# astra-vision/PaSCo

Measured on AMD Instinct MI355X. Metric: scenes/sec (256x256x32, ~10% occ) PaSCo MIMO-3, higher is better.
Workload: dtype f32 (conv products as 3 x f16 split MFMA, fp32 accumulate)

## Files before the change

### pasco_amd/csrc/conv_dma.hip

```cpp
#include <mutex>
#include <stdlib.h>

#include <hip/hip_runtime.h>
#include "ph_common.h"
#ifdef PH_DEV
__device__ unsigned long long g_dma_trace[64 * 8];
#define DMA_STAMP(i)                                                                                              \
  do {                                                                                                            \
    if ((a.ablate & 0x80) && threadIdx.x == 0 && blockIdx.x < 64 && blockIdx.y == 0)                              \
      g_dma_trace[blockIdx.x * 8 + (i)] = __builtin_readcyclecounter();                                           \
  } while (0)
#else
#define DMA_STAMP(i) do { } while (0)
#endif
#define H2_STAMP(i) DMA_STAMP(i)
#include "conv_h2_common.h"

#ifdef PH_DEV
extern "C" int ph_dma_trace_read(unsigned long long *host_out) {
  return hipMemcpyFromSymbol(host_out, HIP_SYMBOL(g_dma_trace), sizeof(g_dma_trace)) == hipSuccess ? 0 : 2;
}
#endif
constexpr int DMA_DENSE_KVOL = 100;
constexpr int DMA_KMAX = 32;
// ... 38 lines not shown
  const int cout = a.cout;
  const int nchunks = a.cpad >> 5;
  const int kper = (a.kvol + a.ksplit - 1) / a.ksplit;
  int k_begin = (int)blockIdx.y * kper;
  const int k_end = (k_begin + kper < a.kvol) ? k_begin + kper : a.kvol;
  int kcount = k_end > k_begin ? k_end - k_begin : 0;
  int kstride = 1;
  if (a.kvol > DMA_DENSE_KVOL && a.tile_k == nullptr && a.ksplit > 1 && !PH_ABLATE(a, 4)) {
    kstride = a.ksplit;
    k_begin = (int)blockIdx.y;
    kcount = k_begin < a.kvol ? (a.kvol - k_begin + kstride - 1) / kstride : 0;
  }
  if (a.tile_k != nullptr) {
    k_begin = a.tile_k[row_tile];
    if (k_begin < 0) return;
    kcount = 1;
  }
  int nstages = kcount * nchunks;
  const uint32_t rsb = 4u * (uint32_t)a.cpad;

  f32x16 acc[TM][TN];
#pragma unroll
  for (int i = 0; i < TM; ++i)
#pragma unroll
    for (int j = 0; j < TN; ++j)
#pragma unroll
      for (int r = 0; r < 16; ++r) acc[i][j][r] = 0.f;

  if (nstages > 0) {
    int *idx_lds = reinterpret_cast<int *>(lds + 2 * STAGE);
    for (int i = tid; i < kcount * BM; i += NT) {
      const int k = i / BM, r = i - k * BM;
      const int64_t row = m0 + r;
      int idx = -1;
      if (row < a.n_out) idx = a.tile_k ? a.nbr[row] : (a.nbr ? a.nbr[(int64_t)(k_begin + k * kstride) * a.nbr_stride + row] : (int)row);
      idx_lds[k * BM + (r % RPP) * 4 + (r / RPP)] = idx;
    }
    asm volatile("s_waitcnt vmcnt(0) lgkmcnt(0)" ::: "memory");
    __builtin_amdgcn_s_barrier();
    DMA_STAMP(7);

    static_assert(BM >= 2 * DMA_KMAX + 4, "the stage list fits one offset slot of the index table");
    int *kmap = idx_lds + (DMA_KMAX - 1) * BM;
    const bool compact = a.kvol > DMA_DENSE_KVOL && a.tile_k == nullptr && !PH_ABLATE(a, 4);
    if (compact) {
      int *kflag = kmap + DMA_KMAX;
      for (int k = wave; k < kcount; k += WAVES) {
        bool any = false;
        for (int r = lane; r < BM; r += 64) any |= idx_lds[k * BM + r] >= 0;
        const unsigned long long bal = __ballot(any);
        if (lane == 0) kflag[k] = bal != 0ull ? 1 : 0;
      }
      asm volatile("s_waitcnt lgkmcnt(0)" ::: "memory");
      __builtin_amdgcn_s_barrier();
      if (tid == 0) {
        int nv = 0;
        for (int k = 0; k < kcount; ++k)
          if (kflag[k]) kmap[nv++] = k;
        kflag[DMA_KMAX] = nv;
      }
      asm volatile("s_waitcnt lgkmcnt(0)" ::: "memory");
      __builtin_amdgcn_s_barrier();
      nstages = kflag[DMA_KMAX] * nchunks;
    }
    if (nstages > 0) {

    const int l_j = tid & 7;
    const int l_r = tid >> 3;
    const uint32_t sj16 = (uint32_t)((l_j ^ ((l_r >> 1) & 7)) << 4);
    const uint64_t in_base = (uint64_t)reinterpret_cast<uintptr_t>(a.in_split) + sj16;
    const uint64_t zero_src = (uint64_t)reinterpret_cast<uintptr_t>(a.zero) + sj16;
    const uint64_t w_base = (uint64_t)reinterpret_cast<uintptr_t>(a.w_split) + sj16;
    uint32_t boff[B_PASSES];
#pragma unroll
    for (int q = 0; q < B_PASSES; ++q) {
      int n = n0 + l_r + q * RPP;
      n = n < cout ? n : cout - 1;
      boff[q] = (uint32_t)n * rsb;
    }
    const int64_t wslab = (int64_t)cout * rsb;
    static_assert(A_PASSES == 4, "one 16-byte index read per thread and stage");
    typedef int i32x4 __attribute__((ext_vector_type(4)));

    auto stage_kc = [&](int s, int &k, uint32_t &coff) {
      const int sc = s < nstages - 1 ? s : nstages - 1;
      const int kk = sc / nchunks;
      coff = (uint32_t)(sc - kk * nchunks) << 7;
      k = compact ? kmap[kk] : kk;
    };
    auto load_idx = [&](int s) {
      int k;
      uint32_t coff;
      stage_kc(s, k, coff);
      return *reinterpret_cast<const i32x4 *>(idx_lds + k * BM + l_r * 4);
    };
    struct Src {
      uint64_t a[A_PASSES];
      uint64_t w;
    };
    auto prep = [&](int s, const i32x4 &idx, Src &src) {
      int k;
      uint32_t coff;
      stage_kc(s, k, coff);
#pragma unroll
      for (int p = 0; p < A_PASSES; ++p) {
        const int ix = idx[p];
        uint64_t v = in_base + (uint64_t)(uint32_t)(ix < 0 ? 0 : ix) * rsb + coff;
        asm volatile("" : "+v"(v));
        src.a[p] = ix >= 0 ? v : zero_src;
      }
      src.w = w_base + (uint64_t)((int64_t)(k_begin + k * kstride) * wslab) + coff;
    };
    auto fire = [&](const Src &src, int buf) {
      char *abuf = lds + buf * STAGE;
#pragma unroll
      for (int p = 0; p < A_PASSES; ++p) {
        char *dst = abuf + (p * RPP + wave * 8) * 128;
        __builtin_amdgcn_global_load_lds((const __attribute__((address_space(1))) void *)(uintptr_t)src.a[p],
                                         (__attribute__((address_space(3))) void *)dst, 16, 0, 0);
      }
#pragma unroll
      for (int q = 0; q < B_PASSES; ++q) {
        char *dst = abuf + A_BYTES + (q * RPP + wave * 8) * 128;
        __builtin_amdgcn_global_load_lds((const __attribute__((address_space(1))) void *)(uintptr_t)(src.w + boff[q]),
                                         (__attribute__((address_space(3))) void *)dst, 16, 0, 0);
      }
    };

    const int sw = (l31 >> 1) & 7;
    uint32_t xo[2][2];
#pragma unroll
    for (int ks = 0; ks < 2; ++ks)
#pragma unroll
      for (int part = 0; part < 2; ++part) xo[ks][part] = (uint32_t)(((part * 4 + ks * 2 + h) ^ sw) << 4);
    const uint32_t arow = (uint32_t)((wm * TM * 32 + l31) * 128);
    const uint32_t brow = (uint32_t)(A_BYTES + (wn * TN * 32 + l31) * 128);

    struct Frag {
      f16x8 ah[2][TM], al[2][TM], bh[2][TN], bl[2][TN];
    };
    auto readfrag = [&](int buf, Frag &f) {
      const char *base = lds + buf * STAGE;
#pragma unroll
      for (int ks = 0; ks < 2; ++ks) {
#pragma unroll
        for (int i = 0; i < TM; ++i) {
          f.ah[ks][i] = *reinterpret_cast<const f16x8 *>(base + arow + i * 4096 + xo[ks][0]);
          f.al[ks][i] = *reinterpret_cast<const f16x8 *>(base + arow + i * 4096 + xo[ks][1]);
        }
#pragma unroll
        for (int j = 0; j < TN; ++j) {
          f.bh[ks][j] = *reinterpret_cast<const f16x8 *>(base + brow + j * 4096 + xo[ks][0]);
          f.bl[ks][j] = *reinterpret_cast<const f16x8 *>(base + brow + j * 4096 + xo[ks][1]);
        }
      }
    };
    auto mfma = [&](const Frag &f) {
#pragma unroll
      for (int ks = 0; ks < 2; ++ks)
#pragma unroll
        for (int i = 0; i < TM; ++i)
#pragma unroll
          for (int j = 0; j < TN; ++j) {
            acc[i][j] = __builtin_amdgcn_mfma_f32_32x32x16_f16(f.bh[ks][j], f.al[ks][i], acc[i][j], 0, 0, 0);
            acc[i][j] = __builtin_amdgcn_mfma_f32_32x32x16_f16(f.bl[ks][j], f.ah[ks][i], acc[i][j], 0, 0, 0);
            acc[i][j] = __builtin_amdgcn_mfma_f32_32x32x16_f16(f.bh[ks][j], f.ah[ks][i], acc[i][j], 0, 0, 0);
          }
    };
    auto fire_mfma = [&](const Src &src, int buf, const Frag &f) {
      char *abuf = lds + buf * STAGE;
// ... 177 lines not shown
```

### pasco_amd/csrc/conv_f16x3.hip

```cpp
#include <stdio.h>
#include <stdlib.h>

#include "conv_h2_common.h"

template <int BM, int KC, int WM, int WN, int TM, int TN>
__global__ void __launch_bounds__(HV_THREADS) k_conv_f16x3(ConvArgsH a) {
  constexpr int BN = WN * TN * 32;
  constexpr int HKC = KC;
  constexpr int H_LD = KC + 8;
  constexpr int A_TPR = KC / 4;
  constexpr int A_RPP = HV_THREADS / A_TPR;
  constexpr int A_PASSES = BM / A_RPP;
  constexpr int B_SPR = KC / 8;
  constexpr int B_SLOTS = (BN * B_SPR + HV_THREADS - 1) / HV_THREADS;
  static_assert(WM * WN == 4 && WM * TM * 32 == BM, "tile shape");
  static_assert(B_SLOTS >= 1, "loader shape");

  __shared__ __attribute__((aligned(16))) _Float16 Ah[BM * H_LD];
  __shared__ __attribute__((aligned(16))) _Float16 Al[BM * H_LD];
  __shared__ __attribute__((aligned(16))) _Float16 Bh[BN * H_LD];
  __shared__ __attribute__((aligned(16))) _Float16 Bl[BN * H_LD];

  const int nwg = gridDim.x;
  const int cpx = nwg >> 3;
// ... 466 lines not shown
    x = h_act(x * (a.epi_scale ? a.epi_scale[c] : 1.f) + (a.epi_shift ? a.epi_shift[c] : 0.f), a.epi_neg);
    if (a.has_tail) {
      x = x * (a.epi2_scale ? a.epi2_scale[c] : 1.f) + (a.epi2_shift ? a.epi2_shift[c] : 0.f);
      x = h_act(x + r4[q], a.res_neg);
    }
    v[q] = x;
  }
  if (a.out) *reinterpret_cast<float4 *>(a.out + t) = make_float4(v[0], v[1], v[2], v[3]);
  if (a.out_split) {
    float sc[4], sh[4];
#pragma unroll
    for (int q = 0; q < 4; ++q) {
      sc[q] = a.osp_scale ? a.osp_scale[col + q] : 1.f;
      sh[q] = a.osp_shift ? a.osp_shift[col + q] : 0.f;
    }
    const bool obad = emit_split4(v, sc, sh, a.osp_has, a.osp_neg, a.act_pow2,
                                  a.out_split + (row * (a.cout >> 5) + (col >> 5)) * 64 + (col & 31));
    if (a.status != nullptr && obad) atomicOr(a.status, 1);
  }
}

static int ph_launch_splitk_epilogue(const ConvArgsH &args, hipStream_t st) {
  const int64_t total = args.n_out * args.cout;
  hipLaunchKernelGGL(k_splitk_epilogue, dim3((unsigned)((total / 4 + 255) / 256)), dim3(256), 0, st, args);
  PH_LAUNCH_CHECK();
  return 0;
}

static int ph_conv_h_launch(const ConvArgsH &a, const ConvStep &s, hipStream_t st) {
  const bool pre = s.kernel == CONV_K_H2;
  ConvKernelFn k = nullptr;
#define PH_H2(KC_, BM_, WM_, WN_, TM_, TN_)                                                                                    \
  (s.emit ? k_conv_h2<BM_, KC_, WM_, WN_, TM_, TN_, true> : k_conv_h2<BM_, KC_, WM_, WN_, TM_, TN_, false>)
#define PH_H_CASE(BM_, WM_, WN_, TM_, TN_)                                                                                     \
  if (s.bm == BM_) {                                                                                                           \
    if (pre) k = s.kc == 64 ? PH_H2(64, BM_, WM_, WN_, TM_, TN_) : PH_H2(32, BM_, WM_, WN_, TM_, TN_);                         \
    else k = s.kc == 64 ? k_conv_f16x3<BM_, 64, WM_, WN_, TM_, TN_> : k_conv_f16x3<BM_, 32, WM_, WN_, TM_, TN_>;               \
  }
  if (s.bn == 32) {
    PH_H_CASE(128, 4, 1, 1, 1);
  } else if (s.bn == 64) {
    PH_H_CASE(128, 4, 1, 1, 2);
    PH_H_CASE(64, 2, 2, 1, 1);
  } else {
    PH_H_CASE(128, 2, 2, 2, 2);
    PH_H_CASE(64, 2, 2, 1, 2);
    PH_H_CASE(32, 1, 4, 1, 1);
  }
#undef PH_H_CASE
#undef PH_H2
  if (k == nullptr) {
    ph_set_error("conv_fwd(f16x3): no kernel for bm=%d bn=%d", s.bm, s.bn);
    return 1;
  }
  return ph_launch_tiles(k, a, s, st);
}

static ConvKnobs conv_knobs_from_env() {
  ConvKnobs k;
  auto on = [](const char *e, bool dflt) { return e == nullptr ? dflt : atoi(e) != 0; };
  if (const char *e = PH_DEV_ENV("PASCO_CONV_DMA")) {
    k.dma_on = atoi(e) != 0;
    k.dma_all = atoi(e) == 2;
  }
  if (const char *e = PH_DEV_ENV("PASCO_CONV_WIN")) {
    k.win_on = atoi(e) != 0;
    k.win_wide = atoi(e) == 2;
  }
  k.wide_on = on(PH_DEV_ENV("PASCO_CONV_WIDE"), true);
  k.mid_on = on(PH_DEV_ENV("PASCO_CONVH_MID"), true);
  k.rl_on = on(PH_DEV_ENV("PASCO_CONV_RL"), true);
  if (const char *e = PH_DEV_ENV("PASCO_CONVH_CFG")) k.has_cfg = sscanf(e, "%d,%d", &k.cfg_bm, &k.cfg_kc) >= 1;
  if (const char *e = PH_DEV_ENV("PASCO_CONVH_KSPLIT")) {
    k.has_ksplit = true;
    k.ksplit = atoi(e);
  }
  k.ksplit_model = on(PH_DEV_ENV("PASCO_CONVH_KSPLIT_MODEL"), true);
  k.tail_on = on(PH_DEV_ENV("PASCO_CONV_TAIL"), true);
  k.dma_inter = on(PH_DEV_ENV("PASCO_CONV_DMA_INTER"), true);
  k.wop2 = on(PH_DEV_ENV("PASCO_WOP"), true);
  if (const char *e = PH_DEV_ENV("PASCO_CONV_LIN")) k.lin_on = atoi(e);
  if (const char *e = PH_DEV_ENV("PASCO_GRID_KS")) k.grid_ks = atoi(e);
  k.grid_upw = on(PH_DEV_ENV("PASCO_GRID_UPW"), true);
  return k;
}
#ifdef PH_DEV
static ConvKnobs &conv_knobs() {
  static ConvKnobs k = conv_knobs_from_env();
  return k;
}
extern "C" void ph_conv_dma_set_ablate(int mask) {
  conv_knobs().dma_ablate = mask & 0xff;
  conv_knobs().dma_tall = (mask & 0x100) != 0;
}
extern "C" void ph_conv_lin_set(int on) { conv_knobs().lin_on = on; }
extern "C" void ph_conv_grid_set_ablate(int mask) { conv_knobs().grid_ablate = mask; }
#else
static const ConvKnobs &conv_knobs() {
  static const ConvKnobs k = conv_knobs_from_env();
  return k;
}
#endif

static ConvArgsH conv_args(const ph_conv_desc *d) {
  ConvArgsH a{};
  a.in = d->in;
  a.w_hi = (const _Float16 *)d->w_f16_hi;
  a.w_lo = (const _Float16 *)d->w_f16_lo;
  a.nbr = d->nbr;
  a.out = d->out;
  a.n_in = d->n_in;
  a.n_out = d->n_out;
  a.cin = d->cin;
  a.cout = d->cout;
  a.kvol = d->kvol;
  a.pro_scale = d->pro_scale;
  a.pro_shift = d->pro_shift;
  a.bias = d->bias;
  a.epi_scale = d->epi_scale;
  a.epi_shift = d->epi_shift;
  a.epi2_scale = d->epi2_scale;
  a.epi2_shift = d->epi2_shift;
  a.residual = d->residual;
  a.pro_neg = neg_of(d->pro_act, d->epi_slope);
  a.epi_neg = neg_of(d->epi_act, d->epi_slope);
  a.res_neg = neg_of(d->res_act, d->epi_slope);
  a.w_unscale = d->w_unscale;
  a.has_pro = (d->pro_scale || d->pro_shift || d->pro_act != PH_ACT_NONE) ? 1 : 0;
  a.has_tail = (d->residual || d->epi2_scale || d->epi2_shift || d->res_act != PH_ACT_NONE || d->axis_table) ? 1 : 0;
  a.status = d->status;
  a.ksplit = 1;
  a.in_split = (const _Float16 *)d->in_split;
  a.w_split = (const _Float16 *)d->w_split;
  a.w_frag = (const _Float16 *)d->w_frag;
  a.cpad = (d->cin + 31) / 32 * 32;
  a.out_split = (_Float16 *)d->out_split;
  a.osp_scale = d->osp_scale;
  a.osp_shift = d->osp_shift;
  a.osp_neg = neg_of(d->osp_act, d->epi_slope);
  a.osp_has = (d->osp_scale || d->osp_shift || d->osp_act != PH_ACT_NONE) ? 1 : 0;
  a.act_pow2 = ldexpf(1.f, d->split_exp2);
  a.route = d->route;
  a.win_rows = d->win_rows;
  a.win_cnt = d->win_cnt;
  a.win_slots = d->win_slots;
  a.axis_table = d->axis_table;
  a.axis_coords = d->axis_coords;
  a.axis_lo = d->axis_lo;
  a.axis_rows = d->axis_rows;
  {
    uintptr_t bits = 0;
    const float *vecs[] = {d->bias, d->epi_scale, d->epi_shift, d->epi2_scale, d->epi2_shift, d->osp_scale, d->osp_shift};
    for (const float *v : vecs) bits |= (uintptr_t)v;
    a.par_vec = ((bits & 15) == 0 && d->cout % 4 == 0) ? 1 : 0;
  }
  a.tail_ws = d->splitk_ws;
  a.tail_ws_bytes = d->splitk_ws_bytes;
  for (int q = 0; q < 4; ++q) a.gdim[q] = d->grid_dims[q];
  for (int q = 0; q < 3; ++q) a.gker[q] = d->grid_kernel[q];
  a.nbr_stride = d->n_out;
  return a;
}

static ConvShape conv_shape(const ph_conv_desc *d, bool have_zero_line) {
  ConvShape s;
  s.mma_mode = d->mma_mode;
  s.n_in = d->n_in, s.n_out = d->n_out;
  s.cin = d->cin, s.cout = d->cout, s.kvol = d->kvol, s.route = d->route;
  s.ws_bytes = d->splitk_ws != nullptr ? d->splitk_ws_bytes : 0;
  s.nbr = d->nbr != nullptr, s.out = d->out != nullptr, s.out_split = d->out_split != nullptr, s.w_frag = d->w_frag != nullptr;
  s.axis = d->axis_table != nullptr, s.residual = d->residual != nullptr;
  s.win = d->win_rows && d->win_cnt && d->win_slots && d->win_stats;
  s.rl = d->rl_in && d->rl_out && d->rl_tile_k;
  s.rl_rows = d->rl_rows;
  for (int q = 0; q < 4; ++q) s.grid_dims[q] = d->grid_dims[q];
  for (int q = 0; q < 3; ++q) s.grid_kernel[q] = d->grid_kernel[q];
  s.have_zero_line = have_zero_line;
  return s;
}

static ConvArgsH step_args(const ConvArgsH &map, const ph_conv_desc *d, const ConvStep &s, const char *zero) {
  ConvArgsH a = row_range(map, s.row0, s.rows);
  if (s.rowlist) {
    a.nbr = d->rl_in;
    a.out_rows = d->rl_out;
    a.tile_k = d->rl_tile_k;
  }
  a.ksplit = s.ksplit;
  a.partial = s.use_ws ? (float *)d->splitk_ws : nullptr;
  a.grid_upw = s.grid_upw;
  if (s.win_pair) {
    a.win_stats = d->win_stats;
    a.win_which = s.win_which;
    a.win_gather = s.win_gather;
  }
  if (s.kernel == CONV_K_DMA || s.kernel == CONV_K_WIDE || s.kernel == CONV_K_WIN || s.kernel == CONV_K_WOP2) a.zero = zero;
  a.ablate = s.ablate;
  if (s.no_axis) a.axis_table = nullptr;
  if (s.no_residual) a.residual = nullptr;
  return a;
}

int ph_conv_fwd_f16x3(const ph_conv_desc *d, hipStream_t st) {
  const bool pre = d->mma_mode == 2;
  PH_REQUIRE(d->cin % 8 == 0 && d->cout % 4 == 0, "conv_fwd(f16x3): needs cin %% 8 == 0 and cout %% 4 == 0");
  if (pre) {
    PH_REQUIRE(d->in_split && d->w_split, "conv_fwd(f16x3, mode 2): pre-split operands missing");
    PH_REQUIRE((((uintptr_t)d->in_split | (uintptr_t)d->w_split) & 15) == 0, "conv_fwd(f16x3): 16-byte alignment");
    PH_REQUIRE(d->n_in < ((int64_t)1 << 31), "conv_fwd(f16x3): n_in too large");
    PH_REQUIRE((((uintptr_t)d->out | (uintptr_t)d->residual | (uintptr_t)d->splitk_ws) & 15) == 0,
               "conv_fwd(f16x3, mode 2): out / residual / splitk_ws must be 16-byte aligned");
  } else {
    PH_REQUIRE(d->w_f16_hi && d->w_f16_lo, "conv_fwd(f16x3): pre-split weights missing");
    PH_REQUIRE((((uintptr_t)d->in | (uintptr_t)d->w_f16_hi | (uintptr_t)d->w_f16_lo) & 15) == 0,
               "conv_fwd(f16x3): 16-byte alignment");
  }
  PH_REQUIRE(d->split_exp2 >= -16 && d->split_exp2 <= 16, "conv_fwd(f16x3): split_exp2 out of range (%d)", d->split_exp2);
  if (d->out_split) {
    PH_REQUIRE(pre, "conv_fwd(f16x3): out_split needs mma_mode 2");
    PH_REQUIRE(d->cout % 32 == 0 && (((uintptr_t)d->out_split) & 15) == 0, "conv_fwd(f16x3): out_split needs cout %% 32 == 0");
  }
  PH_REQUIRE(d->out || d->out_split, "conv_fwd(f16x3): no output buffer");
  if (d->axis_table) {
    PH_REQUIRE(pre, "conv_fwd: axis_table needs mma_mode 2");
    PH_REQUIRE(d->axis_coords && d->axis_rows > 0 && d->cout % 4 == 0 && (((uintptr_t)d->axis_table | (uintptr_t)d->axis_coords) & 15) == 0,
               "conv_fwd: axis_table needs axis_coords, axis_rows > 0, 16-byte alignment");
  }
  const ConvArgsH map = conv_args(d);
  const char *zero = pre ? ph_dma_zero_line() : nullptr;
  const ConvPlan plan = conv_plan(conv_shape(d, zero != nullptr), conv_knobs());
  if (plan.error == CONV_PLAN_NO_ZERO_LINE) {
    ph_set_error("conv_fwd(windows): no zero line");
    return 2;
  }
  for (int i = 0; i < plan.nsteps; ++i) {
    const ConvStep &s = plan.step[i];
    const ConvArgsH a = step_args(map, d, s, zero);
    int rc;
    switch (s.kernel) {
      case CONV_K_DMA: rc = ph_conv_dma_launch(a, s, st); break;
      case CONV_K_WIDE: rc = ph_conv_wide_launch(a, s, st); break;
      case CONV_K_LIN: rc = ph_conv_lin_launch(a, s, st); break;
      case CONV_K_GRID: rc = ph_conv_grid_launch(a, s, st); break;
      case CONV_K_WIN: rc = ph_conv_win_launch(a, s, st); break;
      case CONV_K_WOP2: rc = ph_conv_wop2_launch(a, s, st); break;
      default: rc = ph_conv_h_launch(a, s, st); break;
    }
    if (rc) return rc;
    if (s.ksplit > 1) {
      if (int rc2 = ph_launch_splitk_epilogue(a, st)) return rc2;
    }
  }
  const int *c = plan.cfg;
  ph_record_cfg(c[0], c[1], c[2], c[3], c[4], c[5], c[6], c[7]);
  return 0;
}
```

### pasco_amd/csrc/conv_h2_common.h

```cpp
#pragma once
#include <type_traits>

#include "conv_plan.h"
#include "ph_common.h"

typedef float f32x16 __attribute__((ext_vector_type(16)));
typedef _Float16 f16x8 __attribute__((ext_vector_type(8)));
typedef _Float16 f16x4 __attribute__((ext_vector_type(4)));
typedef unsigned u32x2 __attribute__((ext_vector_type(2)));

constexpr int HV_THREADS = 256;

__device__ __forceinline__ float h_act(float v, float neg) { return ph_act(v, neg); }
__device__ __forceinline__ bool h_out_of_range(float t) { return !(fabsf(t) <= 65504.f); }

struct ConvArgsH {
  const float *in;
  const _Float16 *w_hi;
  const _Float16 *w_lo;
  const int32_t *nbr;
  float *out;
  int64_t n_in, n_out;
  int cin, cout, kvol;
  const float *pro_scale, *pro_shift, *bias, *epi_scale, *epi_shift, *epi2_scale, *epi2_shift, *residual;
  float pro_neg, epi_neg, res_neg, w_unscale;
  int has_pro, has_tail;
  int n_row_tiles, n_col_tiles;
  int32_t *status;
  int ksplit;
  float *partial;
  const _Float16 *in_split;
  const _Float16 *w_split;
  const _Float16 *w_frag;
  int cpad;
  _Float16 *out_split;
  const float *osp_scale, *osp_shift;
  float osp_neg;
  int osp_has;
  float act_pow2;
  const char *zero;
  int ablate;
  int route;
  const int32_t *win_rows, *win_cnt, *win_stats;
  const uint16_t *win_slots;
  int win_which;
  int win_gather;
  const float *axis_table;
  const int32_t *axis_coords;
  int axis_lo, axis_rows;
  const int32_t *out_rows, *tile_k;
  int par_vec;
  void *tail_ws;
  int64_t tail_ws_bytes;
  int gdim[4], gker[3];
  int grid_upw;
  int64_t nbr_stride;
};

__device__ __forceinline__ bool ph_axis_offsets(const ConvArgsH &a, int64_t row, int64_t (&off)[3]) {
  const int4 c = *reinterpret_cast<const int4 *>(a.axis_coords + row * 4);
  const int v[3] = {c.y, c.z, c.w};
  bool clamped = false;
#pragma unroll
  for (int ax = 0; ax < 3; ++ax) {
    int idx = v[ax] - a.axis_lo;
    clamped |= idx < 0 || idx >= a.axis_rows;
    idx = idx < 0 ? 0 : (idx >= a.axis_rows ? a.axis_rows - 1 : idx);
    off[ax] = ((int64_t)ax * a.axis_rows + idx) * a.cout;
  }
  return clamped;
}
__device__ __forceinline__ float4 ph_axis_residual4(const ConvArgsH &a, const int64_t (&off)[3], int col) {
  float4 s = make_float4(0.f, 0.f, 0.f, 0.f);
#pragma unroll
  for (int ax = 0; ax < 3; ++ax) {
    const float4 t = *reinterpret_cast<const float4 *>(a.axis_table + off[ax] + col);
    s.x += t.x; s.y += t.y; s.z += t.z; s.w += t.w;
  }
  return s;
}
__device__ __forceinline__ float4 ph_axis_residual4(const ConvArgsH &a, int64_t row, int col) {
  int64_t off[3];
  ph_axis_offsets(a, row, off);
  return ph_axis_residual4(a, off, col);
}
__device__ __forceinline__ void ph_par4(const ConvArgsH &a, const float *p, int col, bool ok, float dflt, float (&dst)[4]) {
  dst[0] = dst[1] = dst[2] = dst[3] = dflt;
  if (p == nullptr || !ok) return;
  if (a.par_vec) {
    const float4 v = *reinterpret_cast<const float4 *>(p + col);
    dst[0] = v.x; dst[1] = v.y; dst[2] = v.z; dst[3] = v.w;
  } else {
#pragma unroll
    for (int q = 0; q < 4; ++q) dst[q] = p[col + q];
  }
}

__device__ __forceinline__ bool ph_win_pred(const int32_t *stats, int which, int64_t n_row_tiles) {
  if (which & 0x100) return true;
  if (which & 0x200) return false;
  return (int64_t)stats[which & 1] * 4 <= n_row_tiles * 5;
}
const char *ph_dma_zero_line();
int ph_conv_dma_launch(const ConvArgsH &a, const ConvStep &s, hipStream_t st);
int ph_conv_lin_launch(const ConvArgsH &a, const ConvStep &s, hipStream_t st);
int ph_conv_wide_launch(const ConvArgsH &a, const ConvStep &s, hipStream_t st);
int ph_conv_grid_launch(const ConvArgsH &a, const ConvStep &s, hipStream_t st);
int ph_conv_win_launch(const ConvArgsH &a, const ConvStep &s, hipStream_t st);
int ph_conv_wop2_launch(const ConvArgsH &a, const ConvStep &s, hipStream_t st);

static inline float neg_of(int act, float slope) { return act == PH_ACT_RELU ? 0.f : (act == PH_ACT_LEAKY ? slope : 1.f); }

static inline ConvArgsH row_range(const ConvArgsH &a, int64_t r0, int64_t rows) {
  ConvArgsH v = a;
  v.n_out = rows;
  if (v.nbr) v.nbr = a.nbr + r0;
  if (v.out) v.out = a.out + r0 * a.cout;
  if (v.out_split) v.out_split = a.out_split + r0 * a.cout * 2;
  if (v.residual) v.residual = a.residual + r0 * a.cout;
  if (v.axis_coords) v.axis_coords = a.axis_coords + r0 * 4;
  return v;
}

typedef void (*ConvKernelFn)(ConvArgsH);
static inline int ph_launch_tiles(ConvKernelFn kernel, const ConvArgsH &a, const ConvStep &s, hipStream_t st) {
  ConvArgsH args = a;
  args.n_row_tiles = (int)conv_tiles(a.n_out, s.bm);
  args.n_col_tiles = (int)conv_tiles(a.cout, s.bn);
  const int grid = (args.n_row_tiles * args.n_col_tiles + 7) / 8 * 8;
  hipLaunchKernelGGL(kernel, dim3(grid, s.emit ? 1 : args.ksplit), dim3(s.waves * 64), 0, st, args);
  PH_LAUNCH_CHECK();
  return 0;
}

__device__ __forceinline__ bool emit_split4(const float v[4], const float *sc, const float *sh, int has, float neg,
                                            float pow2, _Float16 *dst) {
  f16x4 hi, lo;
  bool bad = false;
// ... 395 lines not shown
```

### pasco_amd/csrc/conv_plan.h

```cpp
#pragma once
#include <math.h>
#include <stdint.h>

#include "../../include/pasco_hip.h"

enum ConvKernel { CONV_K_F16X3 = 1, CONV_K_H2, CONV_K_DMA, CONV_K_WIN, CONV_K_WOP2, CONV_K_WIDE, CONV_K_LIN, CONV_K_GRID };

constexpr int CONV_DMA_KMAX = 32;
constexpr int CONV_DMA_DENSE_KVOL = 100;
constexpr int CONV_WIDE_KMAX = 27;

struct ConvShape {
  int mma_mode = 2;
  int64_t n_in = 0, n_out = 0;
  int cin = 0, cout = 0, kvol = 1, route = 0;
  int64_t ws_bytes = 0;
  bool nbr = false, out = false, out_split = false, w_frag = false, axis = false, residual = false;
  bool win = false;
  bool rl = false;
  int64_t rl_rows = 0;
  int grid_dims[4] = {0, 0, 0, 0}, grid_kernel[3] = {0, 0, 0};
  bool have_zero_line = true;
};

struct ConvKnobs {
  bool mid_on = true;
  bool has_cfg = false;
  int cfg_bm = 0, cfg_kc = 0;
  bool has_ksplit = false;
  int ksplit = 0;
  bool ksplit_model = true;
  bool dma_on = true;
  bool dma_all = false;
  bool dma_inter = true;
  bool tail_on = true;
  bool wide_on = true;
  bool win_on = true;
  bool win_wide = false;
  bool wop2 = true;
  bool rl_on = true;
  int lin_on = 1;
  int grid_ks = 0;
  bool grid_upw = true;
  int dma_ablate = 0;
  bool dma_tall = false;
  int grid_ablate = 0;
};

struct ConvStep {
  int kernel = 0;
  int bm = 128, bn = 128, kc = 32, waves = 4;
  bool emit = false, inter = false;
  int ksplit = 1;
  bool use_ws = false;
  int64_t row0 = 0, rows = 0;
  bool rowlist = false;
  int grid_upw = 0;
  bool win_pair = false;
  int win_which = 0, win_gather = 0;
  int lin_wpc = 2;
  int ablate = 0;
  bool no_axis = false, no_residual = false;
};

enum ConvPlanError { CONV_PLAN_OK = 0, CONV_PLAN_NO_ZERO_LINE };

struct ConvPlan {
  int nsteps = 0;
  ConvStep step[3];
  int cfg[8] = {0, 0, 0, 0, 0, 0, 0, 0};
  int error = CONV_PLAN_OK;
};

static inline int64_t conv_tiles(int64_t rows, int bm, int64_t ncol = 1) { return (rows + bm - 1) / bm * ncol; }
static inline int conv_kper(int kvol, int ks) { return (kvol + ks - 1) / ks; }
static inline int slices_without_empty(int kvol, int ks) {
  while (ks > 1 && conv_kper(kvol, conv_kper(kvol, ks)) != ks) --ks;
  return ks;
}
static inline bool split_room(int64_t ks, int64_t rows, int cout, int64_t ws_bytes) {
  return ws_bytes > 0 && ks * rows * cout * 4 <= ws_bytes;
}
static inline int conv_dma_kper_max(int kvol) { return CONV_DMA_KMAX - (kvol > CONV_DMA_DENSE_KVOL ? 1 : 0); }

static inline void conv_plan_record(ConvPlan &p, int mode, int bm, int bn, int kc, int ksplit, int emit, int kid, int waves) {
  const int v[8] = {mode, bm, bn, kc, ksplit, emit, kid, waves};
  for (int q = 0; q < 8; ++q) p.cfg[q] = v[q];
}
static inline ConvStep &conv_plan_push(ConvPlan &p, const ConvStep &s) {
  p.step[p.nsteps] = s;
  return p.step[p.nsteps++];
}

static inline bool conv_plan_dma(ConvPlan &p, const ConvShape &sh, const ConvKnobs &kn, ConvStep s, int bn) {
  if (conv_kper(sh.kvol, s.ksplit) > conv_dma_kper_max(sh.kvol)) return false;
  if (!sh.have_zero_line) return false;
  s.kernel = CONV_K_DMA;
  s.kc = 32;
  s.ablate = kn.dma_ablate & 0x85;
  s.no_axis = (kn.dma_ablate & 0x10) != 0;
  s.no_residual = (kn.dma_ablate & 0x40) != 0;
  s.emit = sh.out_split && s.ksplit == 1;
  const int64_t ncol = conv_tiles(sh.cout, bn);
  const bool tall = bn >= 64 && conv_tiles(s.rows, 256, ncol) * s.ksplit >= 2 * 256 && kn.dma_tall;
  auto shape = [&](ConvStep &t, int waves, int bm) {
    t.waves = waves, t.bm = bm, t.bn = bn;
    t.inter = kn.dma_inter && waves == 4;
  };
  auto record = [&](const ConvStep &t) { conv_plan_record(p, 2, t.bm, t.bn, 32, t.ksplit, t.emit ? 1 : 0, 4, t.waves); };
  if (bn != 128 || tall) {
    shape(s, (bn != 32 && tall) ? 8 : 4, (bn != 32 && tall) ? 256 : 128);
    record(conv_plan_push(p, s));
    return true;
  }
  shape(s, 4, 128);
  const int64_t trow = conv_tiles(s.rows, 128);
  const int64_t slots = 512 / ncol;
  const int64_t rounds = trow / slots, rest = trow - rounds * slots;
  if (kn.tail_on && s.ksplit == 1 && !s.rowlist && sh.nbr && sh.kvol >= 8 && !s.win_gather && rounds >= 1 && rest > 0 &&
      2 * rest <= slots && sh.ws_bytes > 0) {
    int ks = (int)(slots / rest);
    if (ks > sh.kvol / 3) ks = sh.kvol / 3;
    if (ks > 16) ks = 16;
    ks = slices_without_empty(sh.kvol, ks);
    const int64_t r0 = (trow - rest) * 128, tail_rows = s.rows - r0;
    if (ks >= 2 && split_room(ks, tail_rows, sh.cout, sh.ws_bytes)) {
      ConvStep head = s, tail = s;
      head.rows = r0;
      tail.row0 = s.row0 + r0, tail.rows = tail_rows;
      tail.ksplit = ks, tail.use_ws = true, tail.emit = false;
      conv_plan_push(p, head);
      record(conv_plan_push(p, tail));
      return true;
    }
  }
  record(conv_plan_push(p, s));
  return true;
}

static inline bool conv_plan_wide(ConvPlan &p, const ConvShape &sh, const ConvKnobs &kn, const ConvStep &in) {
  if ((sh.cout != 256 && sh.cout != 128) || sh.kvol < 8 || in.win_gather || !sh.nbr) return false;
  const int64_t trow = conv_tiles(sh.n_out, 256);
  if (sh.route & PH_ROUTE_WIDE_NEVER) return false;
  ConvStep s = in;
  s.kernel = CONV_K_WIDE;
  s.bm = 256, s.bn = sh.cout, s.kc = 32, s.waves = 8;
  s.ablate = 0;
  s.ksplit = 1, s.use_ws = false;
  auto record = [&](const ConvStep &t) { conv_plan_record(p, 2, 256, t.bn, 32, t.ksplit, t.emit ? 1 : 0, 6, 8); };
  if (!(sh.route & PH_ROUTE_WIDE_ALWAYS)) {
    if (sh.kvol > CONV_WIDE_KMAX) return false;
    if (sh.cout == 256 && trow < 48) return false;
    if (sh.cout == 128) {
      const int64_t rest = trow % 256;
      if (trow >= 256 && rest != 0 && rest < 150 && in.ksplit == 1 && sh.ws_bytes > 0) {
        const int64_t r0 = (trow - rest) * 256, tail_rows = sh.n_out - r0;
        int ks = (int)(512 / conv_tiles(tail_rows, 128));
        if (ks > sh.kvol / 3) ks = sh.kvol / 3;
        if (ks > 12) ks = 12;
        ks = slices_without_empty(sh.kvol, ks);
        if (ks >= 2 && sh.have_zero_line && split_room(ks, tail_rows, sh.cout, sh.ws_bytes)) {
          ConvStep head = s, tail = in;
          head.rows = r0;
          head.emit = sh.out_split;
          conv_plan_push(p, head);
          tail.row0 = r0, tail.rows = tail_rows;
// ... 2 lines not shown
        }
      }
      if (trow < 150 || (rest != 0 && rest < 150)) return false;
    }
  }
  if (!sh.have_zero_line) return false;
  int ks = conv_kper(sh.kvol, CONV_WIDE_KMAX);
  if (trow * ks < 160) {
    int want = (int)((256 + trow / 2) / trow);
    const int kmax = sh.kvol / 3 > 0 ? sh.kvol / 3 : 1;
    if (want > kmax) want = kmax;
    if (want > ks) ks = want;
  }
  if (ks > 1) {
    if (!split_room(ks, sh.n_out, sh.cout, sh.ws_bytes)) return false;
    s.ksplit = ks, s.use_ws = true;
  }
  s.emit = sh.out_split && s.ksplit == 1;
  record(conv_plan_push(p, s));
  return true;
}

static inline double conv_grid_groups(const int *gd, const int *gk) {
  double zavg = 0.0;
  for (int z = 0; z < gd[3]; ++z)
    for (int iz = 0; iz < gk[2]; ++iz) zavg += (z + iz - gk[2] / 2 >= 0 && z + iz - gk[2] / 2 < gd[3]) ? 1.0 : 0.0;
  return gk[0] * zavg / gd[3];
}
static inline bool conv_plan_grid(ConvPlan &p, const ConvShape &sh, const ConvKnobs &kn, int cpad) {
  const int *gd = sh.grid_dims, *gk = sh.grid_kernel;
  if (gd[0] <= 0 || gd[1] <= 0 || gd[2] <= 0 || gd[3] <= 0) return false;
  if (sh.cout % 128 != 0 || sh.axis) return false;
  if (sh.route & PH_ROUTE_GRID_NEVER) return false;
  const int kx = gk[0], ky = gk[1], kz = gk[2];
  if (ky < 3 || ky > 7 || !(kx & 1) || !(ky & 1) || !(kz & 1) || kx * kz > 64 || kx * ky * kz != sh.kvol) return false;
  const int64_t sites = (int64_t)gd[0] * gd[1] * gd[2] * gd[3];
  if (sites != sh.n_out || sites != sh.n_in) return false;
  const int64_t tiles = conv_tiles(sh.n_out, 256, sh.cout / 128);
  const int nchunks = cpad >> 5;
  const double units = conv_grid_groups(gd, gk) * nchunks;
  const double stage_us = 1.0, fixed_us = 8.0;
  int best = 1;
  double best_us = 1e30;
  for (int ks = 1; ks <= 12; ++ks) {
    if (ks > 1 && !split_room(ks, sh.n_out, sh.cout, sh.ws_bytes)) break;
    if (ks > 1 && units / ks < 2.0) break;
    const double rounds = (double)((tiles * ks + 255) / 256);
    double us = rounds * (ceil(units / ks) * ky * stage_us + fixed_us);
    if (ks > 1) us += (double)ks * (double)sh.n_out * sh.cout * 4.0 / 3.0e6 + 5.0;
    if (us < best_us) best_us = us, best = ks;
  }
  if (kn.grid_ks >= 1 && (kn.grid_ks == 1 || split_room(kn.grid_ks, sh.n_out, sh.cout, sh.ws_bytes))) best = kn.grid_ks;
  int grid_upw = 0;
  if (best > 1 && tiles * best <= 256) {
    const int upw = (int)(units / best + 0.5) > 0 ? (int)(units / best + 0.5) : 1;
    int zmax = 0;
    for (int z = 0; z < gd[3]; ++z) {
      int c = 0;
      for (int iz = 0; iz < kz; ++iz) c += (z + iz - kz / 2 >= 0 && z + iz - kz / 2 < gd[3]) ? 1 : 0;
      zmax = c > zmax ? c : zmax;
    }
    const int zreach = zmax + 1 < kz ? zmax + 1 : kz;
    int ksmax = (kx * zreach * nchunks + upw / 2) / upw;
    ksmax = ksmax > 12 ? 12 : ksmax;
    while (ksmax > best && !split_room(ksmax, sh.n_out, sh.cout, sh.ws_bytes)) --ksmax;
    if (kn.grid_upw) {
      if (ksmax > best) best = ksmax;
      grid_upw = upw;
    }
  }
  ConvStep s;
  s.kernel = CONV_K_GRID;
  s.bm = 256, s.bn = 128, s.kc = 32, s.waves = 8;
  s.rows = sh.n_out;
  s.ksplit = best, s.use_ws = best > 1;
  s.grid_upw = grid_upw;
  s.emit = sh.out_split && best == 1;
  s.ablate = kn.grid_ablate;
  conv_plan_push(p, s);
  conv_plan_record(p, 2, 256, 128, 32, best, s.emit ? 1 : 0, 8, 8);
  return true;
}

static inline ConvPlan conv_plan(const ConvShape &sh, const ConvKnobs &kn) {
  ConvPlan p;
  const bool pre = sh.mma_mode == 2;
  const int cpad = (sh.cin + 31) / 32 * 32;
  const int bn = sh.cout <= 32 ? 32 : (sh.cout <= 64 ? 64 : 128);
  const int64_t ncol = conv_tiles(sh.cout, bn);
  const int64_t t128 = conv_tiles(sh.n_out, 128, ncol);
  int bm = 128;
  if (bn >= 64 && t128 < 2 * 256) bm = 64;
  if (bn == 128 && bm == 64 && conv_tiles(sh.n_out, 64, ncol) < 2 * 256) bm = 32;
  int kc = (sh.cin % 64 == 0 && sh.cin >= 256) ? 64 : 32;
  if (pre && kn.mid_on && bn == 128 && sh.cin == 128 && sh.kvol > 1 && t128 < 3 * 256) {
    if (bm == 128) bm = 64;
    kc = 64;
  }
  if (pre && cpad % 64 != 0) kc = 32;
  const bool env = kn.has_cfg;
  if (env) {
    const int em = kn.cfg_bm, ek = kn.cfg_kc;
    if (em == 128 || (em == 64 && bn >= 64) || (em == 32 && bn == 128)) bm = em;
    if (ek == 32 || (ek == 64 && (!pre || cpad % 64 == 0))) kc = ek;
  }
  int ksplit = 1;
  {
    int want = (int)(2048 / (t128 > 0 ? t128 : 1));
    if (want > 8) want = 8;
    if (want > sh.kvol / 4) want = sh.kvol / 4;
    if (kn.ksplit_model && bn == 128 && t128 < 2 * 256 && sh.kvol >= 8 && sh.ws_bytes > 0) {
      const double stage_us = 1.3, fixed_us = 5.0;
      const double nchunks = (double)(cpad / 32);
      int best = 1;
      double best_us = 1e30;
      for (int ks = 1; ks <= 12 && ks <= sh.kvol / 3; ++ks) {
        const int kper = conv_kper(sh.kvol, ks);
        if (kper > conv_dma_kper_max(sh.kvol) || slices_without_empty(sh.kvol, ks) != ks) continue;
        if (ks > 1 && !split_room(ks, sh.n_out, sh.cout, sh.ws_bytes)) continue;
        const double rounds = (double)((t128 * ks + 511) / 512);
        double us = rounds * (kper * nchunks * stage_us + fixed_us);
        if (ks > 1) us += (double)ks * (double)sh.n_out * sh.cout * 4.0 / 3.0e6 + fixed_us;
        if (us < best_us) best_us = us, best = ks;
      }
      want = best;
    }
    if (kn.has_ksplit) want = kn.ksplit;
    const bool room = split_room(want, sh.n_out, sh.cout, sh.ws_bytes);
    if (bn == 128 && t128 < 2 * 256 && want >= 2 && room && !env) {
      bm = 128;
      ksplit = want;
    } else if (kn.has_ksplit && want >= 2 && room) {
      ksplit = want;
    }
  }
  ConvStep base;
  base.rows = sh.n_out;
  base.bn = bn;
  if (pre && !env && sh.grid_dims[0] > 0 && sh.nbr && conv_plan_grid(p, sh, kn, cpad)) return p;
  if (pre && !env && sh.rl && sh.rl_rows > 0 && kn.rl_on && (bn == 64 || bn == 128)) {
    ConvStep s = base;
    s.rowlist = true;
    s.rows = sh.rl_rows;
    if (conv_plan_dma(p, sh, kn, s, bn)) {
      conv_plan_record(p, 2, 128, bn, 32, 1, sh.out_split ? 1 : 0, 3, 4);
      return p;
    }
  }
  ConvStep g = base;
  g.ksplit = ksplit, g.use_ws = ksplit > 1;
  if (pre && kn.win_on && !env && sh.kvol == 27 &&
      (bn == 64 || (bn == 128 && (kn.win_wide || (sh.route & PH_ROUTE_WIN_ALWAYS)))) && ksplit == 1 && sh.win) {
    if (!sh.have_zero_line) {
      p.error = CONV_PLAN_NO_ZERO_LINE;
      return p;
    }
    ConvStep w = base;
    w.win_pair = true;
    w.win_which = (bn == 64 ? 0 : 1) |
                  ((sh.route & PH_ROUTE_WIN_ALWAYS) ? 0x100 : ((sh.route & PH_ROUTE_WIN_NEVER) ? 0x200 : 0));
    w.win_gather = 0;
    w.emit = sh.out_split;
    w.ablate = kn.dma_ablate;
    w.kc = 32;
    w.kernel = (bn == 64 && kn.wop2 && sh.cout <= 64 && sh.w_frag) ? CONV_K_WOP2 : CONV_K_WIN;
    w.waves = (bn == 64) ? 4 : 8;
    conv_plan_push(p, w);
    g.win_pair = true;
    g.win_which = w.win_which;
    g.win_gather = 1;
    bm = 128;
  }
  const bool pair = g.win_pair;
  auto finish = [&]() -> ConvPlan & {
    if (pair) conv_plan_record(p, 2, 128, bn, 32, 1, sh.out_split ? 1 : 0, 5, 4);
    return p;
  };
  if (pre && kn.wide_on && !env && bn == 128 && (sh.cout == 256 || sh.cout == 128) && sh.kvol >= 8 && sh.nbr &&
      conv_plan_wide(p, sh, kn, g))
    return finish();
  if (pre && kn.dma_on && !env && bn == 128 && sh.kvol == 1 && ksplit == 1 && (kn.lin_on & 1) && !(sh.route & PH_ROUTE_LIN_NEVER) &&
      (cpad == 64 || cpad == 128) && sh.n_out >= 1) {
    ConvStep s = g;
    s.kernel = CONV_K_LIN;
    s.bm = 32, s.bn = 128, s.kc = 32, s.waves = 4;
    s.emit = sh.out_split;
    s.lin_wpc = ((kn.lin_on >> 8) & 15) ? ((kn.lin_on >> 8) & 15) : 2;
    conv_plan_push(p, s);
    conv_plan_record(p, 2, 32, 128, 32, 1, s.emit ? 1 : 0, 7, 4);
    return finish();
  }
  if (pre && kn.dma_on && !env && (bn == 128 || kn.dma_all)) {
    ConvStep s = g;
    if (bm != 128) {
      int want = (int)(1024 / (t128 > 0 ? t128 : 1));
      if (want > 8) want = 8;
      if (want > sh.kvol / 4) want = sh.kvol / 4;
      if (t128 < 256 && want >= 2 && split_room(want, sh.n_out, sh.cout, sh.ws_bytes)) s.ksplit = want, s.use_ws = true;
    }
    if (conv_plan_dma(p, sh, kn, s, bn)) return finish();
  }
  g.kernel = pre ? CONV_K_H2 : CONV_K_F16X3;
  g.bm = bm, g.kc = kc, g.waves = 4;
  g.emit = pre && sh.out_split && ksplit == 1;
  conv_plan_push(p, g);
  conv_plan_record(p, pre ? 2 : 1, bm, bn, kc, ksplit, g.emit ? 1 : 0, pre ? 2 : 1, 4);
  return finish();
}
```

### pasco_amd/csrc/conv_wide.hip

```cpp
#include <stdlib.h>

#include "conv_h2_common.h"

constexpr int WIDE_KMAX = 27;
static_assert(WIDE_KMAX == CONV_WIDE_KMAX, "the planner (conv_plan.h) sizes the slices for this index table");

template <int TN, bool EMIT>
__global__ void __launch_bounds__(512, 2) k_conv_wide(ConvArgsH a) {
  constexpr int WM = 4, WN = 2, TM = 2;
  constexpr int NT = 512;
  constexpr int BM = WM * TM * 32;
  constexpr int BN = WN * TN * 32;
  constexpr int RPP = NT / 8;
  constexpr int A_BYTES = BM * 128, B_BYTES = BN * 128, STAGE = A_BYTES + B_BYTES;
  constexpr int A_PASSES = BM / RPP, B_PASSES = BN / RPP;
  constexpr int L = A_PASSES + B_PASSES;
  constexpr int NMH = TM * TN * 3;
  constexpr int NRH = (TM + TN) * 2;
  static_assert(A_PASSES == 4 && (L == 8 || L == 6), "one 16-byte index read per thread and stage");
  __shared__ __attribute__((aligned(128))) char lds[2 * STAGE + WIDE_KMAX * BM * 4];

  const int nwg = gridDim.x;
  const int cpx = nwg >> 3;
  const int bid = blockIdx.x;
  const int tile = (bid & 7) * cpx + (bid >> 3);
  if (tile >= a.n_row_tiles * a.n_col_tiles) return;
  const int row_tile = tile / a.n_col_tiles;
  const int col_tile = tile - row_tile * a.n_col_tiles;
  const int64_t m0 = (int64_t)row_tile * BM;
  const int n0 = col_tile * BN;

  const int tid = threadIdx.x;
  const int lane = tid & 63;
  const int wave = tid >> 6;
  const int wm = wave / WN, wn = wave % WN;
  const int h = lane >> 5;
  const int l31 = lane & 31;

  const int cout = a.cout;
  const int nchunks = a.cpad >> 5;
  const int kper = (a.kvol + a.ksplit - 1) / a.ksplit;
  const int k_begin = (int)blockIdx.y * kper;
  const int k_end = (k_begin + kper < a.kvol) ? k_begin + kper : a.kvol;
  const int kcount = k_end > k_begin ? k_end - k_begin : 0;
  const int nstages = kcount * nchunks;
  const uint32_t rsb = 4u * (uint32_t)a.cpad;

  f32x16 acc[TM][TN];
#pragma unroll
  for (int i = 0; i < TM; ++i)
#pragma unroll
    for (int j = 0; j < TN; ++j)
#pragma unroll
      for (int r = 0; r < 16; ++r) acc[i][j][r] = 0.f;

  if (nstages > 0) {
    int *idx_lds = reinterpret_cast<int *>(lds + 2 * STAGE);
    for (int i = tid; i < kcount * BM; i += NT) {
      const int k = i / BM, r = i - k * BM;
      const int64_t row = m0 + r;
      int idx = -1;
      if (row < a.n_out) idx = a.nbr ? a.nbr[(int64_t)(k_begin + k) * a.nbr_stride + row] : (int)row;
      idx_lds[k * BM + (r % RPP) * A_PASSES + (r / RPP)] = idx;
    }
    asm volatile("s_waitcnt vmcnt(0) lgkmcnt(0)" ::: "memory");
    __builtin_amdgcn_s_barrier();

    const int l_j = tid & 7;
    const int l_r = tid >> 3;
    const uint32_t sj16 = (uint32_t)((l_j ^ ((l_r >> 1) & 7)) << 4);
    const uint64_t in_base = (uint64_t)reinterpret_cast<uintptr_t>(a.in_split) + sj16;
    const uint64_t zero_src = (uint64_t)reinterpret_cast<uintptr_t>(a.zero) + sj16;
    const uint64_t w_base = (uint64_t)reinterpret_cast<uintptr_t>(a.w_split) + sj16;
    uint32_t boff[B_PASSES];
#pragma unroll
    for (int q = 0; q < B_PASSES; ++q) {
      int n = n0 + l_r + q * RPP;
      n = n < cout ? n : cout - 1;
      boff[q] = (uint32_t)n * rsb;
    }
    const int64_t wslab = (int64_t)cout * rsb;
    typedef int i32x4 __attribute__((ext_vector_type(4)));

    auto stage_kc = [&](int s, int &k, uint32_t &coff) {
      const int sc = s < nstages - 1 ? s : nstages - 1;
      k = sc / nchunks;
      coff = (uint32_t)(sc - k * nchunks) << 7;
    };
    struct Src {
      uint64_t a[A_PASSES];
      uint64_t w;
    };
    auto prep = [&](int s, Src &src) {
      int k;
      uint32_t coff;
      stage_kc(s, k, coff);
      const i32x4 idx = *reinterpret_cast<const i32x4 *>(idx_lds + k * BM + l_r * A_PASSES);
#pragma unroll
      for (int p = 0; p < A_PASSES; ++p) {
        const int ix = idx[p];
        uint64_t v = in_base + (uint64_t)(uint32_t)(ix < 0 ? 0 : ix) * rsb + coff;
        asm volatile("" : "+v"(v));
        src.a[p] = ix >= 0 ? v : zero_src;
      }
      src.w = w_base + (uint64_t)((int64_t)(k_begin + k) * wslab) + coff;
    };
    auto dma_one = [&](const Src &src, char *sbuf, int t) {
      if (t < A_PASSES) {
        char *dst = sbuf + (t * RPP + wave * 8) * 128;
        __builtin_amdgcn_global_load_lds((const __attribute__((address_space(1))) void *)(uintptr_t)src.a[t],
                                         (__attribute__((address_space(3))) void *)dst, 16, 0, 0);
      } else {
        const int q = t - A_PASSES;
        char *dst = sbuf + A_BYTES + (q * RPP + wave * 8) * 128;
        __builtin_amdgcn_global_load_lds((const __attribute__((address_space(1))) void *)(uintptr_t)(src.w + boff[q]),
                                         (__attribute__((address_space(3))) void *)dst, 16, 0, 0);
      }
    };
    auto fire_all = [&](const Src &src, char *sbuf) {
#pragma unroll
      for (int t = 0; t < L; ++t) dma_one(src, sbuf, t);
    };

    const int sw = (l31 >> 1) & 7;
    uint32_t xo[2][2];
#pragma unroll
    for (int ks = 0; ks < 2; ++ks)
#pragma unroll
      for (int part = 0; part < 2; ++part) xo[ks][part] = (uint32_t)(((part * 4 + ks * 2 + h) ^ sw) << 4);
    const uint32_t arow = (uint32_t)((wm * TM * 32 + l31) * 128);
    const uint32_t brow = (uint32_t)(A_BYTES + (wn * TN * 32 + l31) * 128);
    struct Frag {
      f16x8 ah[2][TM], al[2][TM], bh[2][TN], bl[2][TN];
    };
    Frag f;
    auto read_one = [&](const char *base, int ks, int r) {
      if (r < 2 * TM) {
        const int i = r >> 1;
        if ((r & 1) == 0) f.ah[ks][i] = *reinterpret_cast<const f16x8 *>(base + arow + i * 4096 + xo[ks][0]);
        else f.al[ks][i] = *reinterpret_cast<const f16x8 *>(base + arow + i * 4096 + xo[ks][1]);
      } else {
        const int j = (r - 2 * TM) >> 1;
        if (((r - 2 * TM) & 1) == 0) f.bh[ks][j] = *reinterpret_cast<const f16x8 *>(base + brow + j * 4096 + xo[ks][0]);
        else f.bl[ks][j] = *reinterpret_cast<const f16x8 *>(base + brow + j * 4096 + xo[ks][1]);
      }
    };
    auto mfma_one = [&](int ks, int m) {
      const int ij = m % (TM * TN), p = m / (TM * TN);
      const int i = ij / TN, j = ij % TN;
      if (p == 0) acc[i][j] = __builtin_amdgcn_mfma_f32_32x32x16_f16(f.bh[ks][j], f.al[ks][i], acc[i][j], 0, 0, 0);
      else if (p == 1) acc[i][j] = __builtin_amdgcn_mfma_f32_32x32x16_f16(f.bl[ks][j], f.ah[ks][i], acc[i][j], 0, 0, 0);
      else acc[i][j] = __builtin_amdgcn_mfma_f32_32x32x16_f16(f.bh[ks][j], f.ah[ks][i], acc[i][j], 0, 0, 0);
    };
    Src src;
    auto half_a = [&](const char *cur) {
#pragma unroll
      for (int g = 0; g < NRH; ++g) {
        read_one(cur, 1, g);
        __builtin_amdgcn_sched_barrier(0);
#pragma unroll
        for (int m = g * NMH / NRH; m < (g + 1) * NMH / NRH; ++m) mfma_one(0, m);
        __builtin_amdgcn_sched_barrier(0);
      }
    };
    auto half_b = [&](char *cur, const char *nxt, int s) {
#pragma unroll
      for (int g = 0; g < NRH; ++g) {
        if (g < L) dma_one(src, cur, g);
        read_one(nxt, 0, g);
        if (g == L) prep(s + 3, src);
        __builtin_amdgcn_sched_barrier(0);
#pragma unroll
        for (int m = g * NMH / NRH; m < (g + 1) * NMH / NRH; ++m) mfma_one(1, m);
        __builtin_amdgcn_sched_barrier(0);
      }
    };

    char *b0 = lds, *b1 = lds + STAGE;
    prep(0, src);
    fire_all(src, b0);
    prep(1, src);
    fire_all(src, b1);
    prep(2, src);
    if (L == 8) asm volatile("s_waitcnt vmcnt(8)" ::: "memory");
    else asm volatile("s_waitcnt vmcnt(6)" ::: "memory");
    __builtin_amdgcn_s_barrier();
#pragma unroll
    for (int r = 0; r < NRH; ++r) read_one(b0, 0, r);
    asm volatile("s_waitcnt lgkmcnt(0)" ::: "memory");
#define WIDE_MIDDLE()                                           \
  do {                                                          \
    asm volatile("s_waitcnt vmcnt(0) lgkmcnt(0)" ::: "memory"); \
    __builtin_amdgcn_s_barrier();                               \
  } while (0)
    for (int s = 0; s < nstages; s += 2) {
      half_a(b0);
      WIDE_MIDDLE();
      half_b(b0, b1, s);
      asm volatile("s_waitcnt lgkmcnt(0)" ::: "memory");
      if (s + 1 >= nstages) break;
      half_a(b1);
      WIDE_MIDDLE();
      half_b(b1, b0, s + 1);
      asm volatile("s_waitcnt lgkmcnt(0)" ::: "memory");
    }
    asm volatile("s_waitcnt vmcnt(0)" ::: "memory");
#undef WIDE_MIDDLE
  }

  h2_store_tile<TM, TN, EMIT>(a, acc, m0, n0, wm, wn, h, l31);
}

int ph_conv_wide_launch(const ConvArgsH &a, const ConvStep &s, hipStream_t st) {
  const ConvKernelFn k = s.bn == 256 ? (s.emit ? k_conv_wide<4, true> : k_conv_wide<4, false>)
                                     : (s.emit ? k_conv_wide<2, true> : k_conv_wide<2, false>);
  return ph_launch_tiles(k, a, s, st);
}
```

Measured before the change: 49.67.

## Add chunk-outer stage ordering for DMA and wide sparse conv kernels

Adds an option to iterate the reduction stages with the input-channel chunk as the outer loop and kernel offset as the inner loop, instead of offset-outer. In the wide kernel this uses a templated path that advances the weight pointer incrementally rather than dividing per stage. The planner enables it by default only for kvol=27, cin=cout=128 layers on the wide/DMA kernels. The intent is to change gather/weight access locality across stages (e.g. reuse of weight slabs or input rows in cache), at the cost of extra template instantiations and a different accumulation order.

```diff
diff --git a/pasco_amd/csrc/conv_dma.hip b/pasco_amd/csrc/conv_dma.hip
--- a/pasco_amd/csrc/conv_dma.hip
+++ b/pasco_amd/csrc/conv_dma.hip
@@ -144,10 +144,13 @@
     static_assert(A_PASSES == 4, "one 16-byte index read per thread and stage");
     typedef int i32x4 __attribute__((ext_vector_type(4)));
 
+    const bool couter = a.chunk_outer && !compact && a.tile_k == nullptr;
+    const int sdiv = couter ? kcount : nchunks;
     auto stage_kc = [&](int s, int &k, uint32_t &coff) {
       const int sc = s < nstages - 1 ? s : nstages - 1;
-      const int kk = sc / nchunks;
-      coff = (uint32_t)(sc - kk * nchunks) << 7;
+      const int q = sc / sdiv, r = sc - q * sdiv;
+      const int kk = couter ? r : q;
+      coff = (uint32_t)(couter ? q : r) << 7;
       k = compact ? kmap[kk] : kk;
     };
     auto load_idx = [&](int s) {
diff --git a/pasco_amd/csrc/conv_f16x3.hip b/pasco_amd/csrc/conv_f16x3.hip
--- a/pasco_amd/csrc/conv_f16x3.hip
+++ b/pasco_amd/csrc/conv_f16x3.hip
@@ -572,6 +572,7 @@
   if (const char *e = PH_DEV_ENV("PASCO_CONV_LIN")) k.lin_on = atoi(e);
   if (const char *e = PH_DEV_ENV("PASCO_GRID_KS")) k.grid_ks = atoi(e);
   k.grid_upw = on(PH_DEV_ENV("PASCO_GRID_UPW"), true);
+  if (const char *e = PH_DEV_ENV("PASCO_CONV_CHUNK_OUTER")) k.chunk_outer = atoi(e) < 0 ? -1 : (atoi(e) != 0 ? 1 : 0);
   return k;
 }
 #ifdef PH_DEV
@@ -585,6 +586,7 @@
 }
 extern "C" void ph_conv_lin_set(int on) { conv_knobs().lin_on = on; }
 extern "C" void ph_conv_grid_set_ablate(int mask) { conv_knobs().grid_ablate = mask; }
+extern "C" void ph_conv_set_chunk_outer(int v) { conv_knobs().chunk_outer = v < 0 ? -1 : (v != 0 ? 1 : 0); }
 #else
 static const ConvKnobs &conv_knobs() {
   static const ConvKnobs k = conv_knobs_from_env();
@@ -679,6 +681,7 @@
   a.ksplit = s.ksplit;
   a.partial = s.use_ws ? (float *)d->splitk_ws : nullptr;
   a.grid_upw = s.grid_upw;
+  a.chunk_outer = s.chunk_outer ? 1 : 0;
   if (s.win_pair) {
     a.win_stats = d->win_stats;
     a.win_which = s.win_which;
diff --git a/pasco_amd/csrc/conv_h2_common.h b/pasco_amd/csrc/conv_h2_common.h
--- a/pasco_amd/csrc/conv_h2_common.h
+++ b/pasco_amd/csrc/conv_h2_common.h
@@ -54,6 +54,7 @@
   int64_t tail_ws_bytes;
   int gdim[4], gker[3];
   int grid_upw;
+  int chunk_outer;
   int64_t nbr_stride;
 };
 
diff --git a/pasco_amd/csrc/conv_plan.h b/pasco_amd/csrc/conv_plan.h
--- a/pasco_amd/csrc/conv_plan.h
+++ b/pasco_amd/csrc/conv_plan.h
@@ -45,6 +45,7 @@
   int dma_ablate = 0;
   bool dma_tall = false;
   int grid_ablate = 0;
+  int chunk_outer = -1;
 };
 
 struct ConvStep {
@@ -59,6 +60,7 @@
   bool win_pair = false;
   int win_which = 0, win_gather = 0;
   int lin_wpc = 2;
+  bool chunk_outer = false;
   int ablate = 0;
   bool no_axis = false, no_residual = false;
 };
@@ -82,6 +84,13 @@
   return ws_bytes > 0 && ks * rows * cout * 4 <= ws_bytes;
 }
 static inline int conv_dma_kper_max(int kvol) { return CONV_DMA_KMAX - (kvol > CONV_DMA_DENSE_KVOL ? 1 : 0); }
+
+static inline bool conv_can_chunk_outer(int kvol, int cpad, int bn, bool rowlist, bool grid) {
+  return bn == 128 && kvol >= 8 && kvol <= CONV_WIDE_KMAX && cpad >= 64 && !rowlist && !grid;
+}
+static inline bool conv_chunk_outer(int kvol, int cpad, int cout, bool rowlist, bool grid) {
+  return conv_can_chunk_outer(kvol, cpad, cout > 64 ? 128 : 64, rowlist, grid) && kvol == 27 && cpad == 128 && cout == 128;
+}
 
 static inline void conv_plan_record(ConvPlan &p, int mode, int bm, int bn, int kc, int ksplit, int emit, int kid, int waves) {
   const int v[8] = {mode, bm, bn, kc, ksplit, emit, kid, waves};
@@ -250,7 +259,7 @@
   return true;
 }
 
-static inline ConvPlan conv_plan(const ConvShape &sh, const ConvKnobs &kn) {
+static inline ConvPlan conv_plan_routes(const ConvShape &sh, const ConvKnobs &kn) {
   ConvPlan p;
   const bool pre = sh.mma_mode == 2;
   const int cpad = (sh.cin + 31) / 32 * 32;
@@ -375,3 +384,16 @@
   conv_plan_record(p, pre ? 2 : 1, bm, bn, kc, ksplit, g.emit ? 1 : 0, pre ? 2 : 1, 4);
   return finish();
 }
+static inline ConvPlan conv_plan(const ConvShape &sh, const ConvKnobs &kn) {
+  ConvPlan p = conv_plan_routes(sh, kn);
+  const int cpad = (sh.cin + 31) / 32 * 32;
+  const int bn = sh.cout <= 32 ? 32 : (sh.cout <= 64 ? 64 : 128);
+  for (int i = 0; i < p.nsteps; ++i) {
+    ConvStep &s = p.step[i];
+    if (s.kernel != CONV_K_WIDE && s.kernel != CONV_K_DMA) continue;
+    const bool grid = sh.grid_dims[0] > 0;
+    s.chunk_outer = kn.chunk_outer >= 0 ? kn.chunk_outer != 0 && conv_can_chunk_outer(sh.kvol, cpad, bn, s.rowlist, grid)
+                                        : conv_chunk_outer(sh.kvol, cpad, sh.cout, s.rowlist, grid);
+  }
+  return p;
+}
diff --git a/pasco_amd/csrc/conv_wide.hip b/pasco_amd/csrc/conv_wide.hip
--- a/pasco_amd/csrc/conv_wide.hip
+++ b/pasco_amd/csrc/conv_wide.hip
@@ -5,7 +5,7 @@
 constexpr int WIDE_KMAX = 27;
 static_assert(WIDE_KMAX == CONV_WIDE_KMAX, "the planner (conv_plan.h) sizes the slices for this index table");
 
-template <int TN, bool EMIT>
+template <int TN, bool EMIT, bool CO>
 __global__ void __launch_bounds__(512, 2) k_conv_wide(ConvArgsH a) {
   constexpr int WM = 4, WN = 2, TM = 2;
   constexpr int NT = 512;
@@ -82,10 +82,23 @@
     const int64_t wslab = (int64_t)cout * rsb;
     typedef int i32x4 __attribute__((ext_vector_type(4)));
 
-    auto stage_kc = [&](int s, int &k, uint32_t &coff) {
-      const int sc = s < nstages - 1 ? s : nstages - 1;
-      k = sc / nchunks;
-      coff = (uint32_t)(sc - k * nchunks) << 7;
+    int wk = 0;
+    uint32_t wcoff = 0;
+    uint64_t wuni = (uint64_t)((int64_t)k_begin * wslab);
+    const uint64_t wwrap = (uint64_t)((int64_t)kcount * wslab) - 128u;
+    auto stage_kc = [&](int s, int &k, uint32_t &coff, uint64_t &woff) {
+      if (CO) {
+        k = wk, coff = wcoff, woff = wuni;
+        if (s < nstages - 1) {
+          wuni += (uint64_t)wslab;
+          if (++wk == kcount) wk = 0, wcoff += 128, wuni -= wwrap;
+        }
+      } else {
+        const int sc = s < nstages - 1 ? s : nstages - 1;
+        k = sc / nchunks;
+        coff = (uint32_t)(sc - k * nchunks) << 7;
+        woff = (uint64_t)((int64_t)(k_begin + k) * wslab) + coff;
+      }
     };
     struct Src {
       uint64_t a[A_PASSES];
@@ -94,7 +107,8 @@
     auto prep = [&](int s, Src &src) {
       int k;
       uint32_t coff;
-      stage_kc(s, k, coff);
+      uint64_t woff;
+      stage_kc(s, k, coff, woff);
       const i32x4 idx = *reinterpret_cast<const i32x4 *>(idx_lds + k * BM + l_r * A_PASSES);
 #pragma unroll
       for (int p = 0; p < A_PASSES; ++p) {
@@ -103,7 +117,7 @@
         asm volatile("" : "+v"(v));
         src.a[p] = ix >= 0 ? v : zero_src;
       }
-      src.w = w_base + (uint64_t)((int64_t)(k_begin + k) * wslab) + coff;
+      src.w = w_base + woff;
     };
     auto dma_one = [&](const Src &src, char *sbuf, int t) {
       if (t < A_PASSES) {
@@ -212,7 +226,12 @@
 }
 
 int ph_conv_wide_launch(const ConvArgsH &a, const ConvStep &s, hipStream_t st) {
-  const ConvKernelFn k = s.bn == 256 ? (s.emit ? k_conv_wide<4, true> : k_conv_wide<4, false>)
-                                     : (s.emit ? k_conv_wide<2, true> : k_conv_wide<2, false>);
+  ConvKernelFn k;
+#define WIDE_CASE(CO)                                                                                   \
+  k = s.bn == 256 ? (s.emit ? k_conv_wide<4, true, CO> : k_conv_wide<4, false, CO>)                     \
+                  : (s.emit ? k_conv_wide<2, true, CO> : k_conv_wide<2, false, CO>)
+  if (a.chunk_outer) WIDE_CASE(true);
+  else WIDE_CASE(false);
+#undef WIDE_CASE
   return ph_launch_tiles(k, a, s, st);
 }
```

Result: slower. 47.09 (-5.2%).
